# Jutho/KrylovKit.jl

Hardware: NVIDIA H100
Metric: eigsolve_lanczos_operator_applications_per_sec (higher is better)
Workload: dtype f64

## Files before the change

krylovkit.jl_b200/csrc/basis.cu:

```cuda
#include "tsk.cuh"
#include <cmath>
#include <algorithm>

int32_t b2k_enqueue_dot(b2k_ctx* ctx, const void* q, void* x, int64_t n, const void* qprev,
                        int sprev_slot, int slot, int accum_slot);
int32_t b2k_enqueue_axpy_dev(b2k_ctx* ctx, void* x, const void* q, int s_slot, int64_t n);
int32_t b2k_enqueue_apply(b2k_ctx* ctx, const b2k_op* op, const VecRef& x, const VecRef& y,
                          double a0, double a1, bool shifted, const VecRef* dotv, int dot_slot);

using namespace tsk;

namespace {


template <typename T, bool UPDATE, bool PROJECT>
__global__ void __launch_bounds__(NTHREADS, 1)
k_phase(const __grid_constant__ PhaseParams<T> p, const __grid_constant__ ColList cl) {
    extern __shared__ __align__(128) uint8_t smem[];
    SmemView sm(smem);
    const int64_t ntiles = (p.n + Cfg<T>::R - 1) / Cfg<T>::R;
    const bool ragged = (p.n % Cfg<T>::R) != 0 && ((ntiles - 1) % gridDim.x) == blockIdx.x;
    pipe_setup(sm, ragged);
    Pipe st;
    if (threadIdx.x >= NCONS) producer_phase<T>(p, cl, sm, st);
    else consumer_phase<T, UPDATE, PROJECT>(p, sm, st);
}

template <typename T>
struct FusedParams {
    PhaseParams<T> ph[3];
    int32_t kind[3];
    int32_t nph;
    unsigned* barrier;
    unsigned barrier_base;
    const int* stop;
    FinalizeParams fin;
    PeerStep ps;
    unsigned long long* trace;
};

template <typename T>
__device__ __forceinline__ void peer_boundary(const FusedParams<T>& fp, int i, uint8_t* smem) {
    __threadfence();
    asm volatile("fence.proxy.async;" ::: "memory");
    __syncthreads();
    int* flag = reinterpret_cast<int*>(smem + OFF_RED + 256);
    if (threadIdx.x == 0) {
        const unsigned old = atomicAdd(fp.barrier, 1u);
        *flag = (old == fp.barrier_base + (unsigned)(i + 1) * gridDim.x - 1u);
    }
    __syncthreads();
    const PeerDev& pd = fp.ps.pd;
    const int tid = threadIdx.x;
    if (fp.ph[i].part_h == nullptr) {
        const unsigned long long sq = fp.ps.seq_norm;
        if (*flag && tid < 32) {
            __threadfence();
            double a = (tid < 16) ? partial_lane_sum(fp.ph[i].part_n, gridDim.x, 1, tid, 16) : 0.0;
            for (int o = 8; o > 0; o >>= 1) a += __shfl_xor_sync(0xffffffffu, a, o);
            if (tid == 0) peer_publish1(pd, PEER_CH_NORM, sq, a);
        }
        peer_wait(pd, PEER_CH_NORM, sq, tid);
        __syncthreads();
        return;
    }
    const unsigned long long seq = fp.ps.seq_coef[i];
    if (*flag && tid < NCONS) {
        __threadfence();
        const int k = fp.ph[i].k;
        const int L = coef_lanes(k);
        const int j = tid / L, l = tid % L;
        const bool valid = j < k;
        const double a = coef_colsum(fp.ph[i].part_h, gridDim.x, B2K_KSTRIDE, j, l, L, valid);
        if (valid && l == 0)
            for (int p = 0; p < pd.nranks; ++p) peer_slot(pd, p, PEER_CH_COEF, seq, pd.rank)[j] = a;
        __threadfence_system();
        named_bar_sync(1, NCONS);
        if (tid < pd.nranks) st_release_sys_u64(peer_flag(pd, tid, PEER_CH_COEF, seq, pd.rank), seq);
    }
    peer_wait(pd, PEER_CH_COEF, seq, tid);
    __syncthreads();
}

template <typename T>
__global__ void __launch_bounds__(NTHREADS, 1)
k_gs_fused(const __grid_constant__ FusedParams<T> fp, const __grid_constant__ ColList cl) {
    extern __shared__ __align__(128) uint8_t smem[];
    if (fp.stop && *reinterpret_cast<const volatile int*>(fp.stop)) {
        if (threadIdx.x == 0 && fp.nph > 1) atomicAdd(fp.barrier, (unsigned)(fp.nph - 1));
        return;
    }
    SmemView sm(smem);
    const bool tr0 = fp.trace && blockIdx.x == 0 && threadIdx.x == 0;
    if (tr0) b2k_trace(fp.trace, 10);
    const int64_t n = fp.ph[0].n;
    const int64_t ntiles = (n + Cfg<T>::R - 1) / Cfg<T>::R;
    const bool ragged = (n % Cfg<T>::R) != 0 && ((ntiles - 1) % gridDim.x) == blockIdx.x;
    pipe_setup(sm, ragged);
    Pipe st;
    const bool prod = threadIdx.x >= NCONS;
    if (fp.ps.on && fp.ps.seq_alpha && !prod) {
        peer_wait(fp.ps.pd, PEER_CH_ALPHA, fp.ps.seq_alpha, threadIdx.x);
        named_bar_sync(1, NCONS);
    }
    if (tr0) b2k_trace(fp.trace, 11);
    for (int i = 0; i < fp.nph; ++i) {
        if (prod) {
            producer_phase<T>(fp.ph[i], cl, sm, st);
        } else {
            if (fp.kind[i] == 0) consumer_phase<T, false, true>(fp.ph[i], sm, st);
            else if (fp.kind[i] == 1) consumer_phase<T, true, true>(fp.ph[i], sm, st);
            else consumer_phase<T, true, false>(fp.ph[i], sm, st);
        }
        if (tr0) b2k_trace(fp.trace, 12 + i);
        if (i + 1 < fp.nph) {
            if (fp.ps.on) peer_boundary<T>(fp, i, smem);
            else grid_barrier(fp.barrier, fp.barrier_base + (unsigned)(i + 1) * gridDim.x);
            if (tr0) b2k_trace(fp.trace, 15 + i);
        }
    }
    if (fp.fin.enabled && !prod) {
        double* sh = reinterpret_cast<double*>(smem + OFF_RED);
        int* flag = reinterpret_cast<int*>(smem + OFF_RED + 256);
        if (fp.ps.on) __threadfence_system();
        else __threadfence();
        named_bar_sync(1, NCONS);
        if (threadIdx.x == 0) {
            const unsigned t = atomicInc(fp.fin.ticket, gridDim.x - 1);
            *flag = (t == gridDim.x - 1);
        }
        named_bar_sync(1, NCONS);
        if (*flag) {
            __threadfence();
            if (fp.trace && threadIdx.x == 0) b2k_trace(fp.trace, 18);
            finalize_block(fp.fin, threadIdx.x, sh, fp.ps.on ? &fp.ps : nullptr);
            if (fp.trace && threadIdx.x == 0) b2k_trace(fp.trace, 19);
        }
    }
}

__global__ void __launch_bounds__(NCONS)
k_finalize(const double* __restrict__ A, const double* __restrict__ B, const double* __restrict__ N, int G,
           int stride, int k, double* __restrict__ res, int off, int noff) {
    __shared__ double sh[2];
    FinalizeParams f;
    f.A = A; f.B = B; f.N = N; f.G = G; f.stride = stride; f.k = k; f.res = res; f.off = off; f.noff = noff;
    f.rec = nullptr; f.alpha_col = -1; f.tol = 0.0; f.stop = nullptr; f.ticket = nullptr; f.enabled = 1;
    f.peer = 0; f.G_local = G; f.norm_done = 0;
    finalize_block(f, threadIdx.x, sh);
}
// ... 809 lines not shown
            const T a = (T)cf.c[i];
            if (beta_mode == 1) col[r] = fma(a, yv, col[r]);
            else if (beta_mode == 0) col[r] = a * yv;
            else col[r] = fma(a, yv, beta * col[r]);
        }
    }
}


template <typename T, bool U, bool P>
int32_t launch_phase_t(b2k_ctx* ctx, const PhaseParams<T>& p, const ColList& cl, int grid) {
    k_phase<T, U, P><<<grid, NTHREADS, SMEM_BYTES, ctx->stream>>>(p, cl);
    B2K_LAUNCH_CHECK(ctx);
    return B2K_OK;
}

template <typename T>
int32_t launch_phase(b2k_ctx* ctx, const PhaseParams<T>& p, const ColList& cl, int kind, int grid) {
    if (kind == 0) return launch_phase_t<T, false, true>(ctx, p, cl, grid);
    if (kind == 1) return launch_phase_t<T, true, true>(ctx, p, cl, grid);
    return launch_phase_t<T, true, false>(ctx, p, cl, grid);
}

template <typename T>
int grid_for_rows(const b2k_ctx* ctx, int64_t n) {
    int64_t ntiles = (n + Cfg<T>::R - 1) / Cfg<T>::R;
    if (ntiles < 1) ntiles = 1;
    return (int)std::min<int64_t>(ntiles, ctx->num_sms);
}

bool g_coop_launch = true;

template <typename T>
int32_t launch_fused(b2k_ctx* ctx, FusedParams<T>& fp, const ColList& cl, int grid) {
    fp.barrier = ctx->d_sync + 1;
    fp.barrier_base = ctx->barrier_base;
    ctx->barrier_base += (unsigned)(fp.nph - 1) * (unsigned)grid;
    void* args[] = {(void*)&fp, (void*)&cl};
    if (g_coop_launch)
        B2K_CUDA(ctx, cudaLaunchCooperativeKernel((const void*)k_gs_fused<T>, dim3(grid), dim3(NTHREADS),
                                                  args, SMEM_BYTES, ctx->stream));
    else
        k_gs_fused<T><<<grid, NTHREADS, SMEM_BYTES, ctx->stream>>>(fp, cl);
    B2K_LAUNCH_CHECK(ctx);
    return B2K_OK;
}

int32_t enqueue_finalize(b2k_ctx* ctx, const double* A, const double* B, const double* N, int G,
                         int k, int off, int noff) {
    if (k > NCONS) return b2k_fail(ctx, B2K_ENOTSUP, "finalize: more than %d coefficients per pass", NCONS);
    k_finalize<<<1, NCONS, 0, ctx->stream>>>(A, B, N, G, B2K_KSTRIDE, k, ctx->d_res, off, noff);
    B2K_LAUNCH_CHECK(ctx);
    return B2K_OK;
}

bool g_l2_hints = true;
int g_chain_mode = 0;

struct Panel {
    void* base;
    int64_t ld, n;
    int32_t sharded;
    std::vector<int32_t> idx;
};

int32_t make_panel(b2k_ctx* ctx, const b2k_vec* cols, int32_t k, Panel* pn) {
    int32_t sp = 0;
    B2K_TRY(b2k_resolve_cols(ctx, cols, k, &sp, &pn->idx));
    if (k == 0) {
        pn->base = nullptr;
        return B2K_OK;
    }
    const B2kSpace& s = ctx->spaces[sp];
    pn->base = s.base;
    pn->ld = s.ld;
    pn->n = s.n;
    pn->sharded = s.sharded;
    return B2K_OK;
}

template <typename T>
void fill_cols(ColList& cl, const std::vector<int32_t>& idx, int off, int cnt) {
    for (int i = 0; i < cnt; ++i) cl.c[i] = idx[off + i];
}

template <typename T>
PhaseParams<T> base_params(const Panel& pn, int k, const void* x, void* xout) {
    PhaseParams<T> p;
    memset(&p, 0, sizeof(p));
    p.base = (const T*)pn.base;
    p.ld = pn.ld;
    p.n = pn.n;
    p.k = k;
    p.x = (const T*)x;
    p.xout = (T*)xout;
    p.nvec = 1;
    p.beta_mode = 1;
    p.betax = (T)1;
    p.alphac = (T)1;
    p.l2_hints = g_l2_hints ? 1 : 0;
    return p;
}

template <typename T>
int32_t project_t(b2k_ctx* ctx, const Panel& pn, const VecRef& x, int k, int res_off) {
    const int grid = grid_for_rows<T>(ctx, pn.n);
    const int KC = kcap<T>();
    for (int off = 0; off < k; off += KC) {
        const int kk = std::min(KC, k - off);
        ColList cl;
        fill_cols<T>(cl, pn.idx, off, kk);
        PhaseParams<T> p = base_params<T>(pn, kk, x.ptr, nullptr);
        p.part_h = b2k_part_set(ctx, 0);
        const int pr = b2k_prof_begin(ctx, 3, (kk + 1.0) * sizeof(T) * (double)pn.n);
        B2K_TRY((launch_phase_t<T, false, true>(ctx, p, cl, grid)));
        b2k_prof_end(ctx, pr);
        B2K_TRY(enqueue_finalize(ctx, b2k_part_set(ctx, 0), nullptr, nullptr, grid, kk,
                                 res_off + off, 0));
    }
    return B2K_OK;
}

template <typename T>
int32_t unproject_t(b2k_ctx* ctx, const Panel& pn, const VecRef& y, int k, const double* dcoef,
                    const T* coef_t, double alpha, double beta, double* part_n) {
    const int grid = grid_for_rows<T>(ctx, pn.n);
    const int KC = kcap<T>();
    int off = 0;
    do {
// ... 393 lines not shown
            B2K_TRY(b2k_fetch_results(ctx, S_A0 + 1, 0));
            alpha = ctx->h_res[S_A0];
        }
        if (alg == B2K_CGS) {
            B2K_TRY(b2k_vec_axpy2(ctx, w, cols[k - 1], -beta_old, r, -alpha));
            B2K_TRY(b2k_enqueue_dot(ctx, nullptr, rw.ptr, pn.n, nullptr, -1, S_N, -1));
            B2K_TRY(b2k_allreduce(ctx, ctx->d_res + S_N, 1, pn.sharded));
            B2K_TRY(b2k_fetch_results(ctx, S_N + 1, 0));
            *alpha_out = alpha;
            *beta_out = sqrt(ctx->h_res[S_N]);
            return B2K_OK;
        }
        double ab2 = alpha * alpha + beta_old * beta_old;
        double beta = 0.0, nold = 0.0;
        bool first = true;
        for (;;) {
            const bool fusable = fused_ok(ctx, K1, pn.sharded, ctx->dtype);
            const bool prologue = first;
            if (alg == B2K_CGSIR && first) {
                B2K_TRY(b2k_vec_axpy2(ctx, w, cols[k - 1], -beta_old, r, -alpha));
                B2K_TRY(b2k_enqueue_dot(ctx, nullptr, rw.ptr, pn.n, nullptr, -1, S_N, -1));
                B2K_TRY(b2k_allreduce(ctx, ctx->d_res + S_N, 1, pn.sharded));
                B2K_TRY(b2k_fetch_results(ctx, S_N + 1, 0));
                beta = sqrt(ctx->h_res[S_N]);
                nold = sqrt(beta * beta + ab2);
                first = false;
                if (!(eps < beta && beta < eta * nold)) break;
                nold = beta;
                continue;
            }
            if (fusable) {
                const int grid = f64 ? grid_for_rows<double>(ctx, pn.n) : grid_for_rows<float>(ctx, pn.n);
                ColList cl;
                for (int i = 0; i < K1; ++i) cl.c[i] = pn.idx[i];
                double* PA = b2k_part_set(ctx, 0);
                double* PN = b2k_part_set(ctx, 2);
#define BUILD_AND_LAUNCH(T)                                                                   \
    {                                                                                         \
        FusedParams<T> fp;                                                                    \
        memset(&fp, 0, sizeof(fp));                                                           \
        PhaseParams<T> a = base_params<T>(pn, K1, rw.ptr, rw.ptr);                            \
        if (prologue) {                                                                       \
            a.nvec = 3; a.e1 = (const T*)vprev.ptr; a.e2 = (const T*)rv.ptr;                  \
            a.c1 = (T)(-beta_old); a.c2 = (T)(-alpha); a.store_x = 1;                         \
            if (defer_alpha) a.c2_dev = ctx->d_res + S_A0;                                    \
        }                                                                                     \
        a.part_h = PA;                                                                        \
        PhaseParams<T> c = base_params<T>(pn, K1, rw.ptr, rw.ptr);                            \
        c.store_x = 1; c.coef = PA; c.coef_sets = grid; c.coef_stride = B2K_KSTRIDE;          \
        c.alphac = (T)-1; c.part_n = PN;                                                      \
        fp.ph[0] = a; fp.kind[0] = 0; fp.ph[1] = c; fp.kind[1] = 2; fp.nph = 2;               \
        const int pr = b2k_prof_begin(ctx, 1, (2.0 * K1 + 3.0) * sizeof(T) * (double)pn.n);   \
        if (g_use_coop) { B2K_TRY(launch_fused<T>(ctx, fp, cl, grid)); }                      \
        else {                                                                                \
            B2K_TRY(launch_phase<T>(ctx, fp.ph[0], cl, 0, grid));                             \
            B2K_TRY(launch_phase<T>(ctx, fp.ph[1], cl, 2, grid));                             \
        }                                                                                     \
        b2k_prof_end(ctx, pr);                                                                \
    }
                if (f64) BUILD_AND_LAUNCH(double) else BUILD_AND_LAUNCH(float)
#undef BUILD_AND_LAUNCH
                B2K_TRY(enqueue_finalize(ctx, PA, nullptr, PN, grid, K1, S_H, S_N));
                B2K_TRY(b2k_fetch_results(ctx, S_A0 + 1, 0));
                if (defer_alpha) alpha = ctx->h_res[S_A0];
            } else if (one_pass) {
                const int grid = f64 ? grid_for_rows<double>(ctx, pn.n) : grid_for_rows<float>(ctx, pn.n);
                ColList cl;
                for (int i = 0; i < K1; ++i) cl.c[i] = pn.idx[i];
                double* PA = b2k_part_set(ctx, 0);
                double* PN = b2k_part_set(ctx, 2);
#define SPLIT_SWEEPS(T)                                                                       \
    {                                                                                         \
        PhaseParams<T> a = base_params<T>(pn, K1, rw.ptr, rw.ptr);                            \
        if (prologue) {                                                                       \
            a.nvec = 3; a.e1 = (const T*)vprev.ptr; a.e2 = (const T*)rv.ptr;                  \
            a.c1 = (T)(-beta_old); a.c2 = (T)(-alpha); a.store_x = 1;                         \
            if (defer_alpha) a.c2_dev = ctx->d_res + S_A0;                                    \
        }                                                                                     \
        a.part_h = PA;                                                                        \
        const int pr = b2k_prof_begin(ctx, 1, (2.0 * K1 + 3.0) * sizeof(T) * (double)pn.n);   \
        B2K_TRY(launch_phase<T>(ctx, a, cl, 0, grid));                                        \
        B2K_TRY(enqueue_finalize(ctx, PA, nullptr, nullptr, grid, K1, S_H, S_N));             \
        B2K_TRY(b2k_allreduce(ctx, ctx->d_res + S_H, K1, pn.sharded));                        \
        PhaseParams<T> c = base_params<T>(pn, K1, rw.ptr, rw.ptr);                            \
        c.store_x = 1; c.coef = ctx->d_res + S_H; c.coef_sets = 1; c.coef_stride = 0;         \
        c.alphac = (T)-1; c.part_n = PN;                                                      \
        B2K_TRY(launch_phase<T>(ctx, c, cl, 2, grid));                                        \
        b2k_prof_end(ctx, pr);                                                                \
    }
                if (f64) SPLIT_SWEEPS(double) else SPLIT_SWEEPS(float)
#undef SPLIT_SWEEPS
                k_finalize<<<1, NCONS, 0, ctx->stream>>>(PN, nullptr, PN, grid, B2K_KSTRIDE, 0, ctx->d_res, 0, S_N);
                B2K_LAUNCH_CHECK(ctx);
                B2K_TRY(b2k_allreduce(ctx, ctx->d_res + S_N, 1, pn.sharded));
                B2K_TRY(b2k_fetch_results(ctx, S_A0 + 1, 0));
                if (defer_alpha) alpha = ctx->h_res[S_A0];
            } else {
                if (prologue) B2K_TRY(b2k_vec_axpy2(ctx, w, cols[k - 1], -beta_old, r, -alpha));
                if (f64) B2K_TRY(cgs_pass_unfused_t<double>(ctx, pn, rw, K1, S_H, S_N));
                else B2K_TRY(cgs_pass_unfused_t<float>(ctx, pn, rw, K1, S_H, S_N));
                B2K_TRY(b2k_fetch_results(ctx, S_N + 1, 0));
            }
            alpha += ctx->h_res[S_H + k];
            beta = sqrt(ctx->h_res[S_N]);
            first = false;
            if (alg == B2K_CGS2) break;
            if (!(eps < beta && beta < eta * nold)) break;
            nold = beta;
        }
        *alpha_out = alpha;
        *beta_out = beta;
        return B2K_OK;
    }

    B2K_TRY(b2k_enqueue_apply(ctx, op, rv, rw, 0.0, 1.0, false, nullptr, -1));
    B2K_TRY(b2k_vec_axpby(ctx, w, cols[k - 1], -beta_old, 1.0));
    B2K_TRY(b2k_enqueue_dot(ctx, rv.ptr, rw.ptr, pn.n, nullptr, -1, S_A0, -1));
// ... 45 lines not shown
    *beta_out = beta;
    return B2K_OK;
}

bool g_use_chain = true;

bool chain_ok(const b2k_ctx* ctx, const b2k_op* op, const b2k_vec* cols, int32_t k, int32_t nsteps, int32_t alg,
              double beta_old) {
    if (!g_use_chain || !g_use_coop || (alg != B2K_CGS2 && alg != B2K_MGS2B) || nsteps < 1 || nsteps > B2K_MAX_CHAIN)
        return false;
    int64_t op_rows = 0, op_cols = 0;
    int32_t op_kind = -1;
    if (b2k_op_info(op, &op_rows, &op_cols, nullptr, &op_kind) != B2K_OK) return false;
    if ((op_kind != 0 && op_kind != 2) || beta_old == 0.0 || !(beta_old == beta_old)) return false;
    const int32_t sp = B2K_VEC_SPACE(cols[k]);
    if (sp < 0 || sp >= (int32_t)ctx->spaces.size()) return false;
    const B2kSpace& s = ctx->spaces[sp];
    if (ctx->nranks > 1) {
        if (!s.sharded || !b2k_peer_ok(ctx) || !b2k_op_has_peer_halo(op) || op_rows != s.n) return false;
    } else if (op_rows != s.n || op_cols != s.n) {
        return false;
    }
    const int C = ctx->dtype == B2K_F64 ? 8 : 16;
    const int K1 = k + nsteps;
    return (K1 + C - 1) / C <= NS && K1 <= MAXCH * C && K1 <= PEER_SLOT;
}

template <typename T>
int32_t chain_step_gs(b2k_ctx* ctx, const Panel& pn, int K1, const VecRef& rw, const VecRef& vprev,
                      const VecRef& rv, double* rec_prev, double* rec, double tol, const PeerStep* psp,
                      bool scale_after) {
    const int grid = grid_for_rows<T>(ctx, pn.n);
    ColList cl;
    for (int i = 0; i < K1; ++i) cl.c[i] = pn.idx[i];
    double* PA = b2k_part_set(ctx, 0);
    double* PN = b2k_part_set(ctx, 2);
    FusedParams<T> fp;
    memset(&fp, 0, sizeof(fp));
    PhaseParams<T> a = base_params<T>(pn, K1, rw.ptr, rw.ptr);
    a.nvec = 3; a.e1 = (const T*)vprev.ptr; a.e2 = (const T*)rv.ptr; a.store_x = 1;
    a.c1_dev = rec_prev + 2;
    a.c2_dev = rec + 0;
    a.part_h = PA;
    PhaseParams<T> c = base_params<T>(pn, K1, rw.ptr, rw.ptr);
    c.store_x = 1; c.coef = PA; c.coef_sets = grid; c.coef_stride = B2K_KSTRIDE;
    c.alphac = (T)-1; c.part_n = PN;
    fp.ph[0] = a; fp.kind[0] = 0; fp.ph[1] = c; fp.kind[1] = 2; fp.nph = 2;
    if (scale_after) {
        PhaseParams<T> sc = base_params<T>(pn, 0, rw.ptr, rw.ptr);
        sc.store_x = 1; sc.beta_mode = 2; sc.scale_mode = 1;
        sc.scale_norm = PN; sc.scale_G = grid; sc.scale_stride = 1; sc.scale_tol = tol;
        fp.ph[2] = sc; fp.kind[2] = 2; fp.nph = 3;
    }
    fp.stop = reinterpret_cast<const int*>(ctx->d_sync + B2K_SYNC_STOP);
    fp.trace = ctx->d_trace;
    fp.fin.A = PA; fp.fin.B = nullptr; fp.fin.N = PN; fp.fin.G = grid; fp.fin.stride = B2K_KSTRIDE;
    fp.fin.k = K1; fp.fin.res = nullptr; fp.fin.off = 0; fp.fin.noff = 0; fp.fin.rec = rec;
    fp.fin.alpha_col = K1 - 1; fp.fin.tol = tol;
    fp.fin.stop = reinterpret_cast<int*>(ctx->d_sync + B2K_SYNC_STOP);
    fp.fin.ticket = ctx->d_sync + B2K_SYNC_GSFIN; fp.fin.enabled = 1;
    fp.fin.peer = 0; fp.fin.G_local = grid; fp.fin.norm_done = 0;
    if (psp && psp->on) {
        const PeerStep& ps = *psp;
        fp.ps = ps;
        char* win = b2k_peer_local(ctx);
        auto slot = [&](int ch, unsigned long long seq) {
            return reinterpret_cast<double*>(win + PEER_OFF_SLOTS) + (size_t)((ch * 2 + (int)(seq & 1ull)) * PEER_MAXR) * PEER_SLOT;
        };
        fp.ph[0].c2_dev = slot(PEER_CH_ALPHA, ps.seq_alpha);
        fp.ph[0].c2_sets = ps.pd.nranks;
        fp.ph[0].c2_stride = PEER_SLOT;
        fp.ph[1].coef = slot(PEER_CH_COEF, ps.seq_coef[0]);
        fp.ph[1].coef_sets = ps.pd.nranks;
        fp.ph[1].coef_stride = PEER_SLOT;
        fp.fin.A = fp.ph[1].coef; fp.fin.G = ps.pd.nranks; fp.fin.stride = PEER_SLOT; fp.fin.peer = 1;
        const int last = fp.nph - 1;
        if (scale_after) {
            fp.ph[2].scale_norm = slot(PEER_CH_NORM, ps.seq_norm);
            fp.ph[2].scale_G = ps.pd.nranks;
            fp.ph[2].scale_stride = PEER_SLOT;
            fp.fin.norm_done = 1;
        }
        if (ps.seq_halo) {
            fp.ph[last].send_lo = ps.send_lo;
            fp.ph[last].send_hi = ps.send_hi;
            fp.ph[last].halo_dn = ps.send_lo ? reinterpret_cast<T*>(ps.pd.win[ps.pd.rank - 1] + ps.dn_off) : nullptr;
            fp.ph[last].halo_up = ps.send_hi ? reinterpret_cast<T*>(ps.pd.win[ps.pd.rank + 1] + ps.up_off) : nullptr;
        }
    }
    const int pr = b2k_prof_begin(ctx, 1, (2.0 * K1 + 3.0) * sizeof(T) * (double)pn.n);
    B2K_TRY(launch_fused<T>(ctx, fp, cl, grid));
    b2k_prof_end(ctx, pr);
    return B2K_OK;
}

int32_t lanczos_chain(b2k_ctx* ctx, const b2k_op* op, b2k_vec* cols, int32_t k, int32_t nsteps,
                      double beta_old, double tol, int32_t alg, double* alphas_out, double* betas_out,
                      int32_t* steps_done, b2k_vec* r_out) {
    const bool f64 = ctx->dtype == B2K_F64;
    const int32_t space = B2K_VEC_SPACE(cols[k]);
    double* rec0 = ctx->d_steps;
    int* d_stop = reinterpret_cast<int*>(ctx->d_sync + B2K_SYNC_STOP);
    {
        VecRef t;
// ... 599 lines not shown
```

krylovkit.jl_b200/csrc/tsk.cuh:

```cuda
#pragma once
#include "common.cuh"

namespace tsk {

template <typename T> struct Cfg;
template <> struct Cfg<double> {
    static constexpr int R = 256, C = 8, VEC = 2;
    using V16 = double2;
    __device__ static __forceinline__ void unpack(const double2& v, double* o) { o[0] = v.x; o[1] = v.y; }
};
template <> struct Cfg<float> {
    static constexpr int R = 256, C = 16, VEC = 4;
    using V16 = float4;
    __device__ static __forceinline__ void unpack(const float4& v, float* o) {
        o[0] = v.x; o[1] = v.y; o[2] = v.z; o[3] = v.w;
    }
};

constexpr int NS = 12;
constexpr int NW = 3;
constexpr int NCONS = 256;
constexpr int NPROD = 4;
constexpr int NTHREADS = NCONS + 32 * NPROD;
constexpr int MAXCH = 16;
constexpr int SLOT_BYTES = 16384;
static_assert(NS % NPROD == 0, "a ring slot must always be refilled by the same producer warp");

template <typename T> constexpr int kcap() { return MAXCH * Cfg<T>::C; }

constexpr int OFF_RING = 0;
constexpr int OFF_WRING = NS * SLOT_BYTES;
constexpr int WSLOT_MAX = 3 * 256 * 8;
constexpr int OFF_W1 = OFF_WRING + NW * WSLOT_MAX;
constexpr int OFF_CS = OFF_W1 + 2 * 256 * 8;
constexpr int OFF_RED = OFF_CS + 1024;
constexpr int OFF_BAR = OFF_RED + 512;
constexpr int SMEM_BYTES = OFF_BAR + (2 * NS + 2 * NW) * 8;

struct ColList {
    int32_t c[256];
};

template <typename T>
struct PhaseParams {
    const T* base;
    int64_t ld;
    int64_t n;
    int32_t k;
    const T* x;
    T* xout;
    const T* e1;
    const T* e2;
    T c1, c2;
    const double* c1_dev;
    const double* c2_dev;
    int32_t c2_sets;
    int32_t c2_stride;
    T* halo_dn;
    T* halo_up;
    int64_t send_lo, send_hi;
    int32_t scale_mode;
    const double* scale_norm;
    int32_t scale_G, scale_stride;
    double scale_tol;
    int32_t nvec;
    int32_t store_x;
    int32_t l2_hints;
    const double* coef;
    const T* coef_t;
    int32_t coef_sets;
    int32_t coef_stride;
    T alphac, betax;
    int32_t beta_mode;
    double* part_h;
    double* part_n;
};

struct Pipe {
    uint32_t s = 0, ph = 0, ws = 0, wph = 0;
    uint32_t g = 0;
};

struct SmemView {
    uint8_t* raw;
    uint32_t ring, wring, full, empty, wfull, wempty;
    __device__ explicit SmemView(uint8_t* p) : raw(p) {
        ring = smem_u32(p + OFF_RING);
        wring = smem_u32(p + OFF_WRING);
        full = smem_u32(p + OFF_BAR);
        empty = full + NS * 8;
        wfull = empty + NS * 8;
        wempty = wfull + NW * 8;
    }
};

__device__ __forceinline__ void pipe_setup(const SmemView& sm, bool zero_ring) {
    if (threadIdx.x == 0) {
        for (int i = 0; i < NS; ++i) {
// ... 30 lines not shown
        for (int u = 0; u < 12; ++u) a += t[u];
    }
    for (; g + 3 * L < G; g += 4 * L) {
        const double t0 = __ldcg(P + (size_t)g * stride), t1 = __ldcg(P + (size_t)(g + L) * stride);
        const double t2 = __ldcg(P + (size_t)(g + 2 * L) * stride), t3 = __ldcg(P + (size_t)(g + 3 * L) * stride);
        a += t0; a += t1; a += t2; a += t3;
    }
    for (; g < G; g += L) a += __ldcg(P + (size_t)g * stride);
    return a;
}
__device__ __forceinline__ double coef_colsum(const double* P, int G, int stride, int j, int l, int L,
                                              bool valid) {
    double a = valid ? partial_lane_sum(P + j, G, stride, l, L) : 0.0;
    for (int o = L >> 1; o > 0; o >>= 1) a += __shfl_xor_sync(0xffffffffu, a, o);
    return a;
}

template <typename T>
__device__ __forceinline__ void producer_phase(const PhaseParams<T>& p, const ColList& cl,
                                               const SmemView& sm, Pipe& st) {
    using CF = Cfg<T>;
    constexpr int R = CF::R, C = CF::C;
    const int lane = threadIdx.x & 31;
    const uint32_t me = (threadIdx.x - NCONS) >> 5;
    const int nch = (p.k + C - 1) / C;
    const int64_t ntiles = (p.n + R - 1) / R;
    const uint64_t pol = p.l2_hints ? l2_policy_evict_first() : 0;
    for (int64_t tile = blockIdx.x; tile < ntiles; tile += gridDim.x) {
        const int64_t r0 = tile * R;
        const int rt = (int)((p.n - r0) < R ? (p.n - r0) : R);
        const uint32_t bytes = (uint32_t)((rt * sizeof(T) + 15) & ~(size_t)15);
        if (me == 0) {
            mbar_wait(sm.wempty + 8 * st.ws, st.wph ^ 1);
            if (lane == 0) mbar_expect_tx(sm.wfull + 8 * st.ws, bytes * (uint32_t)p.nvec);
            __syncwarp();
            if (lane < p.nvec) {
                const T* src = (lane == 0) ? p.x : (lane == 1 ? p.e1 : p.e2);
                bulk_g2s(sm.wring + st.ws * (3 * R * (int)sizeof(T)) + lane * R * (int)sizeof(T),
                         src + r0, bytes, sm.wfull + 8 * st.ws);
            }
        }
        if (++st.ws == NW) { st.ws = 0; st.wph ^= 1; }
        for (int c = 0; c < nch; ++c) {
            if ((st.g % NPROD) == me) {
                mbar_wait(sm.empty + 8 * st.s, st.ph ^ 1);
                const int ncol = (p.k - c * C) < C ? (p.k - c * C) : C;
                if (lane == 0) mbar_expect_tx(sm.full + 8 * st.s, bytes * (uint32_t)ncol);
                __syncwarp();
                if (lane < ncol) {
                    const T* src = p.base + (int64_t)cl.c[c * C + lane] * p.ld + r0;
                    if (p.l2_hints)
                        bulk_g2s_hint(sm.ring + st.s * SLOT_BYTES + lane * R * (int)sizeof(T), src, bytes,
                                      sm.full + 8 * st.s, pol);
                    else
                        bulk_g2s(sm.ring + st.s * SLOT_BYTES + lane * R * (int)sizeof(T), src, bytes,
                                 sm.full + 8 * st.s);
                }
            }
            ++st.g;
            if (++st.s == NS) { st.s = 0; st.ph ^= 1; }
        }
    }
}

template <typename T> struct VecOps;
template <> struct VecOps<double> {
    __device__ static __forceinline__ void fma_acc(double& acc, const double2& q, const double2& x) {
        acc = fma(q.x, x.x, acc);
        acc = fma(q.y, x.y, acc);
    }
};
template <> struct VecOps<float> {
    __device__ static __forceinline__ void fma_acc(float& acc, const float4& q, const float4& x) {
        acc = fmaf(q.x, x.x, acc);
        acc = fmaf(q.y, x.y, acc);
        acc = fmaf(q.z, x.z, acc);
        acc = fmaf(q.w, x.w, acc);
    }
};

template <typename T, bool UPDATE, bool PROJECT>
__device__ __forceinline__ void consumer_phase(const PhaseParams<T>& p, const SmemView& sm,
                                               Pipe& st) {
    using CF = Cfg<T>;
    using V16 = typename CF::V16;
    constexpr int R = CF::R, C = CF::C, VEC = CF::VEC;
    constexpr int CPW = C / 8;
    constexpr int NLD = R / (32 * VEC);
    const int tid = threadIdx.x;
    const int lane = tid & 31, w = tid >> 5;
    const int nch = (p.k + C - 1) / C;
    const int64_t ntiles = (p.n + R - 1) / R;
    T* cs = reinterpret_cast<T*>(sm.raw + OFF_CS);
    T* w1 = reinterpret_cast<T*>(sm.raw + OFF_W1);
    double* red = reinterpret_cast<double*>(sm.raw + OFF_RED);

    if (UPDATE) {
        if (p.coef_t) {
            for (int j = tid; j < p.k; j += NCONS) cs[j] = p.alphac * p.coef_t[j];
        } else {
            const int L = coef_lanes(p.k);
            const int j = tid / L, l = tid % L;
            const bool valid = j < p.k;
            const double h = coef_colsum(p.coef, p.coef_sets, p.coef_stride, j, l, L, valid);
            if (valid && l == 0) cs[j] = p.alphac * (T)h;
        }
        named_bar_sync(1, NCONS);
    }

    T acc_h[MAXCH][CPW];
#pragma unroll
    for (int c = 0; c < MAXCH; ++c)
#pragma unroll
        for (int cc = 0; cc < CPW; ++cc) acc_h[c][cc] = (T)0;
    T nrm = (T)0;
    int buf = 0;
    const uint64_t pol_last = p.l2_hints ? l2_policy_evict_last() : 0;
    T betax = p.betax;
    bool do_store = p.store_x != 0;
    if (UPDATE && p.scale_mode) {
        double* shn = reinterpret_cast<double*>(sm.raw + OFF_RED + 128);
        if (tid < 32) {
            double a;
            if (p.scale_stride == 1) {
                a = (tid < 16) ? partial_lane_sum(p.scale_norm, p.scale_G, 1, tid, 16) : 0.0;
                for (int o = 8; o > 0; o >>= 1) a += __shfl_xor_sync(0xffffffffu, a, o);
            } else {
                a = 0.0;
                for (int g = 0; g < p.scale_G; ++g)
                    a += *reinterpret_cast<const volatile double*>(p.scale_norm + (size_t)g * p.scale_stride);
            }
            if (tid == 0) shn[0] = a;
        }
        named_bar_sync(1, NCONS);
        const double beta = sqrt(shn[0]);
        if (beta <= p.scale_tol) do_store = false;
        betax = (T)(1.0 / beta);
    }
    T c1 = p.c1, c2 = p.c2;
    if (p.c1_dev) c1 = (T)(-(*reinterpret_cast<const volatile double*>(p.c1_dev)));
    if (p.c2_dev) {
        double a2 = 0.0;
        const int ns = p.c2_sets > 1 ? p.c2_sets : 1;
        for (int g = 0; g < ns; ++g)
            a2 += *reinterpret_cast<const volatile double*>(p.c2_dev + (size_t)g * p.c2_stride);
        c2 = (T)(-a2);
    }

    for (int64_t tile = blockIdx.x; tile < ntiles; tile += gridDim.x) {
        const int64_t r0 = tile * R;
        const int rt = (int)((p.n - r0) < R ? (p.n - r0) : R);
        mbar_wait(sm.wfull + 8 * st.ws, st.wph);
        const T* wv = reinterpret_cast<const T*>(sm.raw + OFF_WRING) + st.ws * 3 * R;
        T xv = wv[tid];
        if (p.nvec == 3) {
            xv = fma(c1, wv[R + tid], xv);
            xv = fma(c2, wv[2 * R + tid], xv);
        }
        if (tid >= rt) xv = (T)0;
        T acc = xv;
        const uint32_t s0 = st.s, ph0 = st.ph;
        if (UPDATE) {
            acc = (p.beta_mode == 0) ? (T)0 : (p.beta_mode == 1 ? xv : betax * xv);
            for (int c = 0; c < nch; ++c) {
                mbar_wait(sm.full + 8 * st.s, st.ph);
                const T* slot = reinterpret_cast<const T*>(sm.raw + OFF_RING + st.s * SLOT_BYTES);
                const int ncol = (p.k - c * C) < C ? (p.k - c * C) : C;
                if (ncol == C) {
                    T cv[C];
#pragma unroll
                    for (int i = 0; i < C / VEC; ++i)
                        CF::unpack(*reinterpret_cast<const V16*>(cs + c * C + i * VEC), cv + i * VEC);
#pragma unroll
                    for (int jj = 0; jj < C; ++jj) acc = fma(slot[jj * R + tid], cv[jj], acc);
                } else {
                    for (int jj = 0; jj < ncol; ++jj) acc = fma(slot[jj * R + tid], cs[c * C + jj], acc);
                }
                if (!PROJECT) {
                    __syncwarp();
                    if (lane == 0) mbar_arrive(sm.empty + 8 * st.s);
                }
                if (++st.s == NS) { st.s = 0; st.ph ^= 1; }
            }
            if (tid >= rt) acc = (T)0;
        }
        if (do_store && tid < rt) {
            if (p.l2_hints) st_hint(p.xout + r0 + tid, acc, pol_last);
            else p.xout[r0 + tid] = acc;
            if (UPDATE && !PROJECT) {
                const int64_t r = r0 + tid;
                if (p.halo_dn && r < p.send_lo) p.halo_dn[r] = acc;
                if (p.halo_up && r >= p.n - p.send_hi) p.halo_up[r - (p.n - p.send_hi)] = acc;
            }
        }
        if (p.part_n) nrm = fma(acc, acc, nrm);
        if (PROJECT) {
            T* wb = w1 + buf * R;
            wb[tid] = acc;
            named_bar_sync(1, NCONS);
            V16 xr[NLD];
#pragma unroll
            for (int i = 0; i < NLD; ++i)
                xr[i] = *reinterpret_cast<const V16*>(wb + VEC * lane + 32 * VEC * i);
            uint32_t ss = UPDATE ? s0 : st.s, pp = UPDATE ? ph0 : st.ph;
#pragma unroll
            for (int c = 0; c < MAXCH; ++c) {
                if (c < nch) {
                    if (!UPDATE) mbar_wait(sm.full + 8 * ss, pp);
                    const T* slot = reinterpret_cast<const T*>(sm.raw + OFF_RING + ss * SLOT_BYTES);
#pragma unroll
                    for (int cc = 0; cc < CPW; ++cc) {
                        const int cj = cc * 8 + w;
                        if (c * C + cj < p.k) {
                            const T* colp = slot + cj * R;
#pragma unroll
                            for (int i = 0; i < NLD; ++i) {
                                V16 q = *reinterpret_cast<const V16*>(colp + VEC * lane + 32 * VEC * i);
                                VecOps<T>::fma_acc(acc_h[c][cc], q, xr[i]);
                            }
                        }
                    }
                    __syncwarp();
                    if (lane == 0) mbar_arrive(sm.empty + 8 * ss);
                    if (++ss == NS) { ss = 0; pp ^= 1; }
                }
            }
            if (!UPDATE) { st.s = ss; st.ph = pp; }
            buf ^= 1;
        }
        __syncwarp();
        if (lane == 0) mbar_arrive(sm.wempty + 8 * st.ws);
        if (++st.ws == NW) { st.ws = 0; st.wph ^= 1; }
    }

    if (PROJECT) {
#pragma unroll
        for (int c = 0; c < MAXCH; ++c) {
#pragma unroll
            for (int cc = 0; cc < CPW; ++cc) {
                const int j = c * C + cc * 8 + w;
                double v = warp_sum((double)acc_h[c][cc]);
                if (c < nch && j < p.k && lane == 0)
                    p.part_h[(size_t)blockIdx.x * B2K_KSTRIDE + j] = v;
            }
        }
    }
    if (p.part_n) {
        double v = warp_sum((double)nrm);
        if (lane == 0) red[w] = v;
        named_bar_sync(1, NCONS);
        if (tid == 0) {
            double s = 0.0;
#pragma unroll
            for (int i = 0; i < NCONS / 32; ++i) s += red[i];
            p.part_n[blockIdx.x] = s;
        }
    }
}

struct FinalizeParams {
    const double* A;
    const double* B;
    const double* N;
    int G, stride, k;
    double* res;
    int off, noff;
    double* rec;
    int alpha_col;
    double tol;
    int* stop;
    unsigned* ticket;
    int enabled;
    int peer;
    int G_local;
    int norm_done;
};
// ... 22 lines not shown
    double alpha0 = f.rec ? f.rec[0] : 0.0;
    if (f.peer && ps) {
        if (!f.norm_done) {
            if (tid == 0) peer_publish1(ps->pd, PEER_CH_NORM, ps->seq_norm, n2);
            peer_wait(ps->pd, PEER_CH_NORM, ps->seq_norm, tid);
        }
        named_bar_sync(1, NCONS);
        if (tid == 0) {
            n2 = peer_sum1(ps->pd, PEER_CH_NORM, ps->seq_norm, 0);
            if (ps->seq_alpha) alpha0 = peer_sum1(ps->pd, PEER_CH_ALPHA, ps->seq_alpha, 0);
            if (ps->seq_halo) {
                __threadfence_system();
                if (ps->send_lo) st_relaxed_sys_u64(peer_hflag(ps->pd, ps->pd.rank - 1, ps->seq_halo, 1), ps->seq_halo);
                if (ps->send_hi) st_relaxed_sys_u64(peer_hflag(ps->pd, ps->pd.rank + 1, ps->seq_halo, 0), ps->seq_halo);
            }
        }
    }
    if (f.N && tid == 0 && f.res) f.res[f.noff] = n2;
    if (f.rec) {
        named_bar_sync(1, NCONS);
        if (tid == 0) {
            f.rec[0] = alpha0;
            const double alpha = alpha0 + sh[0];
            const double beta = sqrt(n2);
            f.rec[1] = alpha;
            f.rec[2] = beta;
            f.rec[3] = 1.0 / beta;
            f.rec[4] = n2;
            if (f.stop && beta <= f.tol) *f.stop = 1;
        }
    }
}

__device__ __forceinline__ void grid_barrier(unsigned* counter, unsigned target) {
    __threadfence();
    asm volatile("fence.proxy.async;" ::: "memory");
    __syncthreads();
    if (threadIdx.x == 0) {
        atomicAdd(counter, 1u);
        while ((int)(*(volatile unsigned*)counter - target) < 0) {
        }
        __threadfence();
    }
    __syncthreads();
}

}
```

Baseline: 357.2.

## Stream prologue vectors via basis ring and let producers run ahead across grid barrier

```diff
diff --git a/krylovkit.jl_b200/csrc/basis.cu b/krylovkit.jl_b200/csrc/basis.cu
--- a/krylovkit.jl_b200/csrc/basis.cu
+++ b/krylovkit.jl_b200/csrc/basis.cu
@@ -23,7 +23,8 @@
     pipe_setup(sm, ragged);
     Pipe st;
     if (threadIdx.x >= NCONS) producer_phase<T>(p, cl, sm, st);
-    else consumer_phase<T, UPDATE, PROJECT>(p, sm, st);
+    else if (p.prologue) consumer_phase<T, UPDATE, PROJECT, true>(p, sm, st);
+    else consumer_phase<T, UPDATE, PROJECT, false>(p, sm, st);
 }
 
 template <typename T>
@@ -31,6 +32,7 @@
     PhaseParams<T> ph[3];
     int32_t kind[3];
     int32_t nph;
+    int32_t run_ahead[2];
     unsigned* barrier;
     unsigned barrier_base;
     const int* stop;
@@ -41,15 +43,16 @@
 
 template <typename T>
 __device__ __forceinline__ void peer_boundary(const FusedParams<T>& fp, int i, uint8_t* smem) {
+    const bool ra = fp.run_ahead[i] != 0;
     __threadfence();
-    asm volatile("fence.proxy.async;" ::: "memory");
-    __syncthreads();
+    if (!ra) asm volatile("fence.proxy.async;" ::: "memory");
+    boundary_sync(ra);
     int* flag = reinterpret_cast<int*>(smem + OFF_RED + 256);
     if (threadIdx.x == 0) {
         const unsigned old = atomicAdd(fp.barrier, 1u);
         *flag = (old == fp.barrier_base + (unsigned)(i + 1) * gridDim.x - 1u);
     }
-    __syncthreads();
+    boundary_sync(ra);
     const PeerDev& pd = fp.ps.pd;
     const int tid = threadIdx.x;
     if (fp.ph[i].part_h == nullptr) {
@@ -61,7 +64,7 @@
             if (tid == 0) peer_publish1(pd, PEER_CH_NORM, sq, a);
         }
         peer_wait(pd, PEER_CH_NORM, sq, tid);
-        __syncthreads();
+        boundary_sync(ra);
         return;
     }
     const unsigned long long seq = fp.ps.seq_coef[i];
@@ -79,7 +82,7 @@
         if (tid < pd.nranks) st_release_sys_u64(peer_flag(pd, tid, PEER_CH_COEF, seq, pd.rank), seq);
     }
     peer_wait(pd, PEER_CH_COEF, seq, tid);
-    __syncthreads();
+    boundary_sync(ra);
 }
 
 template <typename T>
@@ -108,14 +111,22 @@
         if (prod) {
             producer_phase<T>(fp.ph[i], cl, sm, st);
         } else {
-            if (fp.kind[i] == 0) consumer_phase<T, false, true>(fp.ph[i], sm, st);
-            else if (fp.kind[i] == 1) consumer_phase<T, true, true>(fp.ph[i], sm, st);
-            else consumer_phase<T, true, false>(fp.ph[i], sm, st);
+            const PhaseParams<T>& p = fp.ph[i];
+            if (fp.kind[i] == 0) {
+                if (p.prologue) consumer_phase<T, false, true, true>(p, sm, st);
+                else consumer_phase<T, false, true, false>(p, sm, st);
+            } else if (fp.kind[i] == 1) {
+                if (p.prologue) consumer_phase<T, true, true, true>(p, sm, st);
+                else consumer_phase<T, true, true, false>(p, sm, st);
+            } else {
+                if (p.prologue) consumer_phase<T, true, false, true>(p, sm, st);
+                else consumer_phase<T, true, false, false>(p, sm, st);
+            }
         }
         if (tr0) b2k_trace(fp.trace, 12 + i);
-        if (i + 1 < fp.nph) {
+        if (i + 1 < fp.nph && !(prod && fp.run_ahead[i])) {
             if (fp.ps.on) peer_boundary<T>(fp, i, smem);
-            else grid_barrier(fp.barrier, fp.barrier_base + (unsigned)(i + 1) * gridDim.x);
+            else grid_barrier(fp.barrier, fp.barrier_base + (unsigned)(i + 1) * gridDim.x, fp.run_ahead[i] != 0);
             if (tr0) b2k_trace(fp.trace, 15 + i);
         }
     }
@@ -991,7 +1002,24 @@
 bool g_coop_launch = true;
 
 template <typename T>
+bool stores_into_stream(const PhaseParams<T>& st, const PhaseParams<T>& rd, const ColList& cl) {
+    if (!st.store_x || !st.xout) return false;
+    const T* lo = st.xout;
+    const T* hi = st.xout + st.n;
+    auto hits = [&](const T* v) { return v && v < hi && lo < v + rd.n; };
+    if (hits(rd.x)) return true;
+    for (int m = 0; m < rd.k; ++m)
+        if (hits(rd.base + (int64_t)cl.c[m] * rd.ld)) return true;
+    return false;
+}
+
+template <typename T>
 int32_t launch_fused(b2k_ctx* ctx, FusedParams<T>& fp, const ColList& cl, int grid) {
+    for (int i = 0; i + 1 < fp.nph; ++i) {
+        bool ra = true;
+        for (int j = 0; j <= i; ++j) ra = ra && !stores_into_stream<T>(fp.ph[j], fp.ph[i + 1], cl);
+        fp.run_ahead[i] = ra ? 1 : 0;
+    }
     fp.barrier = ctx->d_sync + 1;
     fp.barrier_base = ctx->barrier_base;
     ctx->barrier_base += (unsigned)(fp.nph - 1) * (unsigned)grid;
@@ -1043,6 +1071,11 @@
     for (int i = 0; i < cnt; ++i) cl.c[i] = idx[off + i];
 }
 
+void lanczos_cols(ColList& cl, const Panel& pn, int K1, bool prologue) {
+    const int rot = prologue ? 2 : 0;
+    for (int i = 0; i < K1; ++i) cl.c[(i + rot) % K1] = pn.idx[i];
+}
+
 template <typename T>
 PhaseParams<T> base_params(const Panel& pn, int k, const void* x, void* xout) {
     PhaseParams<T> p;
@@ -1053,7 +1086,6 @@
     p.k = k;
     p.x = (const T*)x;
     p.xout = (T*)xout;
-    p.nvec = 1;
     p.beta_mode = 1;
     p.betax = (T)1;
     p.alphac = (T)1;
@@ -1513,21 +1545,22 @@
             if (fusable) {
                 const int grid = f64 ? grid_for_rows<double>(ctx, pn.n) : grid_for_rows<float>(ctx, pn.n);
                 ColList cl;
-                for (int i = 0; i < K1; ++i) cl.c[i] = pn.idx[i];
+                lanczos_cols(cl, pn, K1, prologue);
                 double* PA = b2k_part_set(ctx, 0);
                 double* PN = b2k_part_set(ctx, 2);
 #define BUILD_AND_LAUNCH(T)                                                                   \
     {                                                                                         \
         FusedParams<T> fp;                                                                    \
         memset(&fp, 0, sizeof(fp));                                                           \
-        PhaseParams<T> a = base_params<T>(pn, K1, rw.ptr, rw.ptr);                            \
+        PhaseParams<T> a = base_params<T>(pn, K1, rw.ptr, nullptr);                           \
+        PhaseParams<T> c = base_params<T>(pn, K1, rw.ptr, rw.ptr);                            \
         if (prologue) {                                                                       \
-            a.nvec = 3; a.e1 = (const T*)vprev.ptr; a.e2 = (const T*)rv.ptr;                  \
-            a.c1 = (T)(-beta_old); a.c2 = (T)(-alpha); a.store_x = 1;                         \
-            if (defer_alpha) a.c2_dev = ctx->d_res + S_A0;                                    \
+            for (PhaseParams<T>* q : {&a, &c}) {                                              \
+                q->prologue = 1; q->c1 = (T)(-beta_old); q->c2 = (T)(-alpha);                 \
+                if (defer_alpha) q->c2_dev = ctx->d_res + S_A0;                               \
+            }                                                                                 \
         }                                                                                     \
         a.part_h = PA;                                                                        \
-        PhaseParams<T> c = base_params<T>(pn, K1, rw.ptr, rw.ptr);                            \
         c.store_x = 1; c.coef = PA; c.coef_sets = grid; c.coef_stride = B2K_KSTRIDE;          \
         c.alphac = (T)-1; c.part_n = PN;                                                      \
         fp.ph[0] = a; fp.kind[0] = 0; fp.ph[1] = c; fp.kind[1] = 2; fp.nph = 2;               \
@@ -1547,23 +1580,24 @@
             } else if (one_pass) {
                 const int grid = f64 ? grid_for_rows<double>(ctx, pn.n) : grid_for_rows<float>(ctx, pn.n);
                 ColList cl;
-                for (int i = 0; i < K1; ++i) cl.c[i] = pn.idx[i];
+                lanczos_cols(cl, pn, K1, prologue);
                 double* PA = b2k_part_set(ctx, 0);
                 double* PN = b2k_part_set(ctx, 2);
 #define SPLIT_SWEEPS(T)                                                                       \
     {                                                                                         \
-        PhaseParams<T> a = base_params<T>(pn, K1, rw.ptr, rw.ptr);                            \
+        PhaseParams<T> a = base_params<T>(pn, K1, rw.ptr, nullptr);                           \
+        PhaseParams<T> c = base_params<T>(pn, K1, rw.ptr, rw.ptr);                            \
         if (prologue) {                                                                       \
-            a.nvec = 3; a.e1 = (const T*)vprev.ptr; a.e2 = (const T*)rv.ptr;                  \
-            a.c1 = (T)(-beta_old); a.c2 = (T)(-alpha); a.store_x = 1;                         \
-            if (defer_alpha) a.c2_dev = ctx->d_res + S_A0;                                    \
+            for (PhaseParams<T>* q : {&a, &c}) {                                              \
+                q->prologue = 1; q->c1 = (T)(-beta_old); q->c2 = (T)(-alpha);                 \
+                if (defer_alpha) q->c2_dev = ctx->d_res + S_A0;                               \
+            }                                                                                 \
         }                                                                                     \
         a.part_h = PA;                                                                        \
         const int pr = b2k_prof_begin(ctx, 1, (2.0 * K1 + 3.0) * sizeof(T) * (double)pn.n);   \
         B2K_TRY(launch_phase<T>(ctx, a, cl, 0, grid));                                        \
         B2K_TRY(enqueue_finalize(ctx, PA, nullptr, nullptr, grid, K1, S_H, S_N));             \
         B2K_TRY(b2k_allreduce(ctx, ctx->d_res + S_H, K1, pn.sharded));                        \
-        PhaseParams<T> c = base_params<T>(pn, K1, rw.ptr, rw.ptr);                            \
         c.store_x = 1; c.coef = ctx->d_res + S_H; c.coef_sets = 1; c.coef_stride = 0;         \
         c.alphac = (T)-1; c.part_n = PN;                                                      \
         B2K_TRY(launch_phase<T>(ctx, c, cl, 2, grid));                                        \
@@ -1675,17 +1709,19 @@
                       bool scale_after) {
     const int grid = grid_for_rows<T>(ctx, pn.n);
     ColList cl;
-    for (int i = 0; i < K1; ++i) cl.c[i] = pn.idx[i];
+    lanczos_cols(cl, pn, K1, true);
     double* PA = b2k_part_set(ctx, 0);
     double* PN = b2k_part_set(ctx, 2);
     FusedParams<T> fp;
     memset(&fp, 0, sizeof(fp));
-    PhaseParams<T> a = base_params<T>(pn, K1, rw.ptr, rw.ptr);
-    a.nvec = 3; a.e1 = (const T*)vprev.ptr; a.e2 = (const T*)rv.ptr; a.store_x = 1;
-    a.c1_dev = rec_prev + 2;
-    a.c2_dev = rec + 0;
+    PhaseParams<T> a = base_params<T>(pn, K1, rw.ptr, nullptr);
+    PhaseParams<T> c = base_params<T>(pn, K1, rw.ptr, rw.ptr);
+    for (PhaseParams<T>* q : {&a, &c}) {
+        q->prologue = 1;
+        q->c1_dev = rec_prev + 2;
+        q->c2_dev = rec + 0;
+    }
     a.part_h = PA;
-    PhaseParams<T> c = base_params<T>(pn, K1, rw.ptr, rw.ptr);
     c.store_x = 1; c.coef = PA; c.coef_sets = grid; c.coef_stride = B2K_KSTRIDE;
     c.alphac = (T)-1; c.part_n = PN;
     fp.ph[0] = a; fp.kind[0] = 0; fp.ph[1] = c; fp.kind[1] = 2; fp.nph = 2;
@@ -1710,9 +1746,11 @@
         auto slot = [&](int ch, unsigned long long seq) {
             return reinterpret_cast<double*>(win + PEER_OFF_SLOTS) + (size_t)((ch * 2 + (int)(seq & 1ull)) * PEER_MAXR) * PEER_SLOT;
         };
-        fp.ph[0].c2_dev = slot(PEER_CH_ALPHA, ps.seq_alpha);
-        fp.ph[0].c2_sets = ps.pd.nranks;
-        fp.ph[0].c2_stride = PEER_SLOT;
+        for (int i = 0; i < 2; ++i) {
+            fp.ph[i].c2_dev = slot(PEER_CH_ALPHA, ps.seq_alpha);
+            fp.ph[i].c2_sets = ps.pd.nranks;
+            fp.ph[i].c2_stride = PEER_SLOT;
+        }
         fp.ph[1].coef = slot(PEER_CH_COEF, ps.seq_coef[0]);
         fp.ph[1].coef_sets = ps.pd.nranks;
         fp.ph[1].coef_stride = PEER_SLOT;
diff --git a/krylovkit.jl_b200/csrc/tsk.cuh b/krylovkit.jl_b200/csrc/tsk.cuh
--- a/krylovkit.jl_b200/csrc/tsk.cuh
+++ b/krylovkit.jl_b200/csrc/tsk.cuh
@@ -49,8 +49,7 @@
     int32_t k;
     const T* x;
     T* xout;
-    const T* e1;
-    const T* e2;
+    int32_t prologue;
     T c1, c2;
     const double* c1_dev;
     const double* c2_dev;
@@ -63,7 +62,6 @@
     const double* scale_norm;
     int32_t scale_G, scale_stride;
     double scale_tol;
-    int32_t nvec;
     int32_t store_x;
     int32_t l2_hints;
     const double* coef;
@@ -160,12 +158,9 @@
         const uint32_t bytes = (uint32_t)((rt * sizeof(T) + 15) & ~(size_t)15);
         if (me == 0) {
             mbar_wait(sm.wempty + 8 * st.ws, st.wph ^ 1);
-            if (lane == 0) mbar_expect_tx(sm.wfull + 8 * st.ws, bytes * (uint32_t)p.nvec);
-            __syncwarp();
-            if (lane < p.nvec) {
-                const T* src = (lane == 0) ? p.x : (lane == 1 ? p.e1 : p.e2);
-                bulk_g2s(sm.wring + st.ws * (3 * R * (int)sizeof(T)) + lane * R * (int)sizeof(T),
-                         src + r0, bytes, sm.wfull + 8 * st.ws);
+            if (lane == 0) {
+                mbar_expect_tx(sm.wfull + 8 * st.ws, bytes);
+                bulk_g2s(sm.wring + st.ws * WSLOT_MAX, p.x + r0, bytes, sm.wfull + 8 * st.ws);
             }
         }
         if (++st.ws == NW) { st.ws = 0; st.wph ^= 1; }
@@ -207,7 +202,7 @@
     }
 };
 
-template <typename T, bool UPDATE, bool PROJECT>
+template <typename T, bool UPDATE, bool PROJECT, bool PRO>
 __device__ __forceinline__ void consumer_phase(const PhaseParams<T>& p, const SmemView& sm,
                                                Pipe& st) {
     using CF = Cfg<T>;
@@ -222,16 +217,15 @@
     T* cs = reinterpret_cast<T*>(sm.raw + OFF_CS);
     T* w1 = reinterpret_cast<T*>(sm.raw + OFF_W1);
     double* red = reinterpret_cast<double*>(sm.raw + OFF_RED);
-
     if (UPDATE) {
         if (p.coef_t) {
-            for (int j = tid; j < p.k; j += NCONS) cs[j] = p.alphac * p.coef_t[j];
+            for (int j = tid; j < p.k; j += NCONS) cs[PRO ? (j + 2) % p.k : j] = p.alphac * p.coef_t[j];
         } else {
             const int L = coef_lanes(p.k);
             const int j = tid / L, l = tid % L;
             const bool valid = j < p.k;
             const double h = coef_colsum(p.coef, p.coef_sets, p.coef_stride, j, l, L, valid);
-            if (valid && l == 0) cs[j] = p.alphac * (T)h;
+            if (valid && l == 0) cs[PRO ? (j + 2) % p.k : j] = p.alphac * (T)h;
         }
         named_bar_sync(1, NCONS);
     }
@@ -279,11 +273,16 @@
         const int64_t r0 = tile * R;
         const int rt = (int)((p.n - r0) < R ? (p.n - r0) : R);
         mbar_wait(sm.wfull + 8 * st.ws, st.wph);
-        const T* wv = reinterpret_cast<const T*>(sm.raw + OFF_WRING) + st.ws * 3 * R;
+        const T* wv = reinterpret_cast<const T*>(sm.raw + OFF_WRING + st.ws * WSLOT_MAX);
         T xv = wv[tid];
-        if (p.nvec == 3) {
-            xv = fma(c1, wv[R + tid], xv);
-            xv = fma(c2, wv[2 * R + tid], xv);
+        T vprev = (T)0, vcur = (T)0;
+        if (PRO) {
+            mbar_wait(sm.full + 8 * st.s, st.ph);
+            const T* slot = reinterpret_cast<const T*>(sm.raw + OFF_RING + st.s * SLOT_BYTES);
+            vprev = slot[tid];
+            vcur = slot[R + tid];
+            xv = fma(c1, vprev, xv);
+            xv = fma(c2, vcur, xv);
         }
         if (tid >= rt) xv = (T)0;
         T acc = xv;
@@ -294,7 +293,8 @@
                 mbar_wait(sm.full + 8 * st.s, st.ph);
                 const T* slot = reinterpret_cast<const T*>(sm.raw + OFF_RING + st.s * SLOT_BYTES);
                 const int ncol = (p.k - c * C) < C ? (p.k - c * C) : C;
-                if (ncol == C) {
+                const int j0 = (PRO && c == 0) ? 2 : 0;
+                if (ncol == C && j0 == 0) {
                     T cv[C];
 #pragma unroll
                     for (int i = 0; i < C / VEC; ++i)
@@ -302,13 +302,17 @@
 #pragma unroll
                     for (int jj = 0; jj < C; ++jj) acc = fma(slot[jj * R + tid], cv[jj], acc);
                 } else {
-                    for (int jj = 0; jj < ncol; ++jj) acc = fma(slot[jj * R + tid], cs[c * C + jj], acc);
+                    for (int jj = j0; jj < ncol; ++jj) acc = fma(slot[jj * R + tid], cs[c * C + jj], acc);
                 }
                 if (!PROJECT) {
                     __syncwarp();
                     if (lane == 0) mbar_arrive(sm.empty + 8 * st.s);
                 }
                 if (++st.s == NS) { st.s = 0; st.ph ^= 1; }
+            }
+            if (PRO) {
+                acc = fma(vprev, cs[0], acc);
+                acc = fma(vcur, cs[1], acc);
             }
             if (tid >= rt) acc = (T)0;
         }
@@ -369,7 +373,7 @@
                 const int j = c * C + cc * 8 + w;
                 double v = warp_sum((double)acc_h[c][cc]);
                 if (c < nch && j < p.k && lane == 0)
-                    p.part_h[(size_t)blockIdx.x * B2K_KSTRIDE + j] = v;
+                    p.part_h[(size_t)blockIdx.x * B2K_KSTRIDE + (PRO ? (j < 2 ? j + p.k - 2 : j - 2) : j)] = v;
             }
         }
     }
@@ -458,17 +462,22 @@
     }
 }
 
-__device__ __forceinline__ void grid_barrier(unsigned* counter, unsigned target) {
+__device__ __forceinline__ void boundary_sync(bool run_ahead) {
+    if (run_ahead) named_bar_sync(1, NCONS);
+    else __syncthreads();
+}
+
+__device__ __forceinline__ void grid_barrier(unsigned* counter, unsigned target, bool run_ahead) {
     __threadfence();
-    asm volatile("fence.proxy.async;" ::: "memory");
-    __syncthreads();
+    if (!run_ahead) asm volatile("fence.proxy.async;" ::: "memory");
+    boundary_sync(run_ahead);
     if (threadIdx.x == 0) {
         atomicAdd(counter, 1u);
         while ((int)(*(volatile unsigned*)counter - target) < 0) {
         }
         __threadfence();
     }
-    __syncthreads();
-}
-
-}
+    boundary_sync(run_ahead);
+}
+
+}
```

New measurement: 369.2 (median of 6 runs). 1.03x the previous value.
